# realphongha/UDP-Pose

Measured on AMD Instinct MI355X. Metric: images/sec HRNet-W32 256x192 (infer+decode), higher is better.
Workload: dtype f16x2 (split fp16 hi+lo operands = 22 bits, 3 fp16 MFMAs per product, fp32 accumulate); 1 GPU; w32 256x192 f16x2 inference, batch=64 per GPU, flip-test on, DARK decode (forward on 2N images + flip fuse + udp_decode_gaussian); global_batch=64, parallelism=replicas x1 (no data-path collective), weights=seeded synthetic, BN stats calibrated (tests/golden/bn_calib_w32_gaussian.npz)

## Files before the change

include/udp_pose_hip.h:

```cpp
#ifndef UDP_POSE_HIP_H
#define UDP_POSE_HIP_H

#include <stddef.h>
#include <stdint.h>

#ifdef __cplusplus
extern "C" {
#endif

#define UDP_POSE_ABI_VERSION 19

enum udp_status {
  UDP_OK = 0,
  UDP_ERR_ARG = -1,
  UDP_ERR_HIP = -2,
  UDP_ERR_UNSUPPORTED = -3,
  UDP_ERR_WORKSPACE = -4
};

enum udp_dtype { UDP_F32 = 0, UDP_BF16 = 1, UDP_F16X2 = 2 };

int udp_abi_version(void);
int udp_f16x2_overflow(void* stream, int reset);
const char* udp_last_error(void);
// ... 109 lines not shown
                          void* w_dgrad, void* stream);
typedef struct udp_pack_desc {
  const float* w;
  void* w_fwd;
  void* w_dgrad;
  int32_t cout, cin, ks, reserved;
} udp_pack_desc;
int udp_pack_conv_weights_batch(const udp_pack_desc* descs_dev, int n, int dtype, void* stream);
int udp_zero_stuff2(const void* dy, int n, int h, int w, int c, int dtype, void* out, void* stream);
size_t udp_conv2d_wgrad_workspace_bytes(int cout, int cin, int ks);
int udp_conv2d_wgrad(const void* x, const void* dy, int n, int hin, int win, int cin_k, int hout,
                     int wout, int cout_k, int ks, int stride, int cout, int cin, int dtype, float* dw,
                     int accumulate, void* workspace, size_t workspace_bytes, void* stream);
typedef struct udp_wgrad_item {
  const void* x;
  const void* dy;
  float* dw;
  void* workspace;
  size_t workspace_bytes;
  int32_t n, hin, win, cin_k, hout, wout, cout_k, ks, stride, cout, cin, accumulate;
} udp_wgrad_item;
int udp_debug_multi_order(const unsigned* tiles, const unsigned* ncby, const int* code, int n, unsigned cap,
                          unsigned* out_member, unsigned* out_tile, unsigned* out_cby, int* used_table);
int udp_conv2d_wgrad_group(const udp_wgrad_item* items, int n_items, int dtype, void* stream);
typedef struct udp_conv_item {
  const udp_conv_op* op;
  const void* in;
  const void* weights;
  const float* bias;
  const void* res;
  void* out;
  double* bn_ws;
  size_t bn_ws_doubles;
  int32_t bn_rows;
  int32_t reserved;
} udp_conv_item;
int udp_conv2d_fused_group(udp_conv_item* items, int n_items, int dtype, int n, void* stream);
size_t udp_bn_workspace_doubles(int c);
int udp_bn_train_fwd(const void* x, int64_t m, int c, const float* gamma, const float* beta, float eps,
                     float momentum, float* running_mean, float* running_var, float* save_mean,
                     float* save_invstd, const void* res, int relu, void* y, int dtype, double* ws,
                     void* stream);
int udp_bn_rows_max(void);
int udp_bn_train_fwd_from_sums(const void* x, int64_t m, int c, const float* gamma, const float* beta, float eps,
                               float momentum, float* running_mean, float* running_var, float* save_mean,
                               float* save_invstd, const void* res, int relu, void* y, int dtype, double* ws,
// ... 67 lines not shown
```

udp-pose_amd/_lib.py:

```python
import ctypes as C
import os

_HERE = os.path.dirname(os.path.abspath(__file__))
LIB_PATH = os.environ.get("UDP_POSE_LIB") or os.path.join(_HERE, "libudp_pose_hip.so")

UDP_OK = 0
UDP_F32, UDP_BF16, UDP_F16X2 = 0, 1, 2
DTYPES = {"f32": UDP_F32, "bf16": UDP_BF16, "f16x2": UDP_F16X2}
UDP_OP_STEM, UDP_OP_CONV, UDP_OP_FUSE, UDP_OP_STEM7, UDP_OP_MAXPOOL, UDP_OP_BILINEAR = 0, 1, 2, 3, 4, 5
UDP_OP_PSA_POOL, UDP_OP_PSA_MLP, UDP_OP_PSA_SCALE, UDP_OP_PSA_SP, UDP_OP_BLOCK = 6, 7, 8, 9, 10
UDP_OP_DECONV, UDP_OP_DWCONV, UDP_OP_PIXSHUF = 11, 12, 13
UDP_BUF_NONE, UDP_BUF_OUTPUT = -1, -2
ABI_VERSION = 19
MAX_LANES, MAX_WAIT = 4, 8


class BnItem(C.Structure):
    _fields_ = [(k, C.c_void_p) for k in ("x", "dy", "y_relu", "res", "y", "dx", "g_out", "gamma", "beta", "running_mean",
                                          "running_var", "save_mean", "save_invstd", "dgamma", "dbeta", "ws")] + [
        ("m", C.c_int64), ("c", C.c_int32), ("rows", C.c_int32), ("relu", C.c_int32), ("reserved", C.c_int32)]


class WgradItem(C.Structure):
    _fields_ = [("x", C.c_void_p), ("dy", C.c_void_p), ("dw", C.c_void_p), ("workspace", C.c_void_p),
# ... 77 lines not shown
                                     C.POINTER(C.c_float), C.POINTER(C.c_float), C.c_int, C.c_int, _P, _P]),
    "udp_aid_apply": (C.c_int, [_P, C.c_int, C.c_int, C.c_int, _P, C.c_int, _P, _P, C.c_int, C.c_int,
                                C.POINTER(C.c_float), C.POINTER(C.c_float), _P]),
    "udp_target_gaussian": (C.c_int, [_P, _P, C.c_int, C.c_int, C.c_int, C.c_int, C.c_int, C.c_int,
                                      C.c_float, _P, _P, _P]),
    "udp_target_offset": (C.c_int, [_P, _P, C.c_int, C.c_int, C.c_int, C.c_int, C.c_int, C.c_int,
                                    C.c_float, _P, _P, _P]),
    "udp_mse_loss": (C.c_int, [_P, _P, _P, C.c_int, C.c_int, C.c_int, C.c_int, _P, _P, _P]),
    "udp_oks_nms": (C.c_int, [_P, _P, _P, _P, C.POINTER(C.c_int32), C.c_int, C.c_int, _P, C.c_double, C.c_int,
                              C.c_double, C.c_int, C.c_double, C.c_int, _P, _P, _P]),
    "udp_pack_conv_weights": (C.c_int, [_P, C.c_int, C.c_int, C.c_int, C.c_int, _P, _P, _P]),
    "udp_pack_conv_weights_batch": (C.c_int, [_P, C.c_int, C.c_int, _P]),
    "udp_zero_stuff2": (C.c_int, [_P, C.c_int, C.c_int, C.c_int, C.c_int, C.c_int, _P, _P]),
    "udp_conv2d_wgrad_workspace_bytes": (C.c_size_t, [C.c_int, C.c_int, C.c_int]),
    "udp_conv2d_wgrad": (C.c_int, [_P, _P] + [C.c_int] * 12 + [_P, C.c_int, _P, C.c_size_t, _P]),
    "udp_bn_workspace_doubles": (C.c_size_t, [C.c_int]),
    "udp_bn_train_fwd": (C.c_int, [_P, C.c_int64, C.c_int, _P, _P, C.c_float, C.c_float, _P, _P, _P, _P, _P,
                                   C.c_int, _P, C.c_int, _P, _P]),
    "udp_bn_rows_max": (C.c_int, []),
    "udp_bn_train_fwd_from_sums": (C.c_int, [_P, C.c_int64, C.c_int, _P, _P, C.c_float, C.c_float, _P, _P, _P, _P, _P,
                                             C.c_int, _P, C.c_int, _P, C.c_int, _P]),
    "udp_bn_train_bwd": (C.c_int, [_P, _P, _P, C.c_int64, C.c_int, _P, _P, _P, _P, _P, _P, _P, C.c_int, _P, _P]),
    "udp_debug_multi_order": (C.c_int, [_P, _P, _P, C.c_int, C.c_uint, _P, _P, _P, _P]),
    "udp_conv2d_wgrad_group": (C.c_int, [_P, C.c_int, C.c_int, _P]),
    "udp_conv2d_fused_group": (C.c_int, [_P, C.c_int, C.c_int, C.c_int, _P]),
    "udp_bn_train_fwd_multi": (C.c_int, [_P, C.c_int, C.c_float, C.c_float, C.c_int, _P]),
    "udp_bn_train_bwd_multi": (C.c_int, [_P, C.c_int, C.c_int, _P]),
    "udp_ew_accumulate": (C.c_int, [_P, _P, C.c_int, C.c_int, C.c_int, C.c_int, C.c_int, C.c_int, C.c_int,
                                    C.c_int, _P]),
    "udp_relu_bwd": (C.c_int, [_P, _P, _P, C.c_int64, C.c_int, _P]),
    "udp_upsample_bwd": (C.c_int, [_P, C.c_int, C.c_int, C.c_int, C.c_int, C.c_int, _P, C.c_int, C.c_int, _P]),
    "udp_bias_grad": (C.c_int, [_P, C.c_int64, C.c_int, C.c_int, _P, C.c_int, _P]),
    "udp_nchw_to_nhwc": (C.c_int, [_P, C.c_int, C.c_int, C.c_int, C.c_int, C.c_int, _P, C.c_int, _P]),
    "udp_adam_step": (C.c_int, [_P, _P, _P, _P, C.c_int64, C.c_float, C.c_float, C.c_float, C.c_float, C.c_int,
                                C.c_float, _P]),
    "udp_adam_coefficients": (C.c_int, [C.c_float, C.c_float, C.c_float, C.c_int, _P]),
    "udp_adam_step_dev": (C.c_int, [_P, _P, _P, _P, C.c_int64, C.c_float, C.c_float, C.c_float, _P, C.c_float, _P]),
    "udp_psa_train_save_floats": (C.c_size_t, [C.c_int, C.c_int, C.c_int, C.c_int]),
    "udp_psa_train_fwd_pool": (C.c_int, [C.POINTER(PsaTrainArgs), C.c_int, _P]),
    "udp_psa_train_fwd_sp": (C.c_int, [C.POINTER(PsaTrainArgs), C.c_int, _P]),
    "udp_psa_train_bwd_sp": (C.c_int, [C.POINTER(PsaTrainArgs), C.c_int, _P]),
    "udp_psa_train_bwd_pool": (C.c_int, [C.POINTER(PsaTrainArgs), C.c_int, _P]),
    "udp_psa_train_bwd_params": (C.c_int, [C.POINTER(PsaTrainArgs), C.c_int, _P]),
}
EXPORTS = tuple(_SIGS)

# ... 42 lines not shown
```

udp-pose_amd/csrc/conv_dev.h:

```cpp
#pragma once
#include <cstdlib>
#include <type_traits>

#include "common.h"

namespace udp {


typedef float f32x4 __attribute__((ext_vector_type(4)));
typedef float f32x2 __attribute__((ext_vector_type(2)));
typedef __bf16 bf16x8 __attribute__((ext_vector_type(8)));
typedef __bf16 bf16x4 __attribute__((ext_vector_type(4)));
typedef _Float16 f16x8 __attribute__((ext_vector_type(8)));
typedef _Float16 f16x4 __attribute__((ext_vector_type(4)));

#ifndef UDP_H2_STORE_AUX
#define UDP_H2_STORE_AUX 0
#endif
#ifndef UDP_H2_RES_AUX
#define UDP_H2_RES_AUX 0
#endif
#ifndef UDP_H2_DMA_AUX
#define UDP_H2_DMA_AUX 0
#endif
// ... 237 lines not shown
      __builtin_amdgcn_raw_buffer_store_b128(__builtin_bit_cast(u32x4, v[nb]), r, voff + 16 * nb, 0, 0);
  } else if constexpr (std::is_same<T, H2>::value) {
#pragma unroll
    for (int h = 0; h < NB / 2; ++h) {
      f16x8 hi, lo;
      h2_split8(v[2 * h], v[2 * h + 1], hi, lo);
      __builtin_amdgcn_raw_buffer_store_b128(__builtin_bit_cast(u32x4, hi), r, voff + 16 * h, 0, UDP_H2_STORE_AUX);
      __builtin_amdgcn_raw_buffer_store_b128(__builtin_bit_cast(u32x4, lo), r, voff + lo_off + 16 * h, 0, UDP_H2_STORE_AUX);
    }
  } else {
#pragma unroll
    for (int h = 0; h < NB / 2; ++h) {
      bf16x8 o;
#pragma unroll
      for (int q = 0; q < 4; ++q) {
        o[q] = (__bf16)v[2 * h][q];
        o[4 + q] = (__bf16)v[2 * h + 1][q];
      }
      __builtin_amdgcn_raw_buffer_store_b128(__builtin_bit_cast(u32x4, o), r, voff + 16 * h, 0, 0);
    }
  }
}

static inline int largest_divisor_leq(int n, int lim) {
  for (int d = lim < n ? lim : n; d >= 1; --d)
    if (n % d == 0) return d;
  return 1;
}

}
```

udp-pose_amd/csrc/conv_ws.hip:

```cpp
#include "conv_dev.h"

namespace udp {

template <int NB>
struct ResH2 {
  u32x4 hi[NB / 2], lo[NB / 2];
};
template <int NB>
__device__ __forceinline__ void load_res_h2(ResH2<NB>& o, __amdgpu_buffer_rsrc_t r, unsigned voff, unsigned lo_off) {
#pragma unroll
  for (int h = 0; h < NB / 2; ++h) {
    o.hi[h] = __builtin_amdgcn_raw_buffer_load_b128(r, voff + 16 * h, 0, UDP_H2_RES_AUX);
    o.lo[h] = __builtin_amdgcn_raw_buffer_load_b128(r, voff + lo_off + 16 * h, 0, UDP_H2_RES_AUX);
  }
}
template <int NB>
__device__ __forceinline__ void add_res_h2(f32x4 (&v)[NB], const ResH2<NB>& o) {
#pragma unroll
  for (int h = 0; h < NB / 2; ++h) h2_add8(v[2 * h], v[2 * h + 1], __builtin_bit_cast(f16x8, o.hi[h]), __builtin_bit_cast(f16x8, o.lo[h]));
}

template <int KS, int STRIDE, int PB, int CP, bool NCHW, bool OUT2 = false>
__device__ __forceinline__ void conv_ws_body(const ConvParams& p, const int tile_id, const int cby) {
  using T = H2;
  constexpr int CK = 32, ESZ = 2, NB = 2, NW = 4;
  constexpr int PAD = KS / 2, TAPS = KS * KS;
  extern __shared__ __attribute__((aligned(16))) unsigned char smem[];

  UDP_STAMP(0);
  const int tid = threadIdx.x;
  const int lane = tid & 63;
  const int wave = __builtin_amdgcn_readfirstlane(tid >> 6);
  const int li = lane & 15;
  const int kg = lane >> 4;
  const int cp = wave % CP, pg = wave / CP;

  int t = tile_id;
  const int tx = t % p.tiles_x;
  t /= p.tiles_x;
  const int ty = t % p.tiles_y;
  const int n0 = (t / p.tiles_y) * p.G;
  const int y0 = ty * p.R;
  const int x0 = tx * p.TW;

  const int IH = p.IH, IW = p.IW;
  const int npix_in = p.G * IH * IW;
  const int in_groups = (npix_in + 15) >> 4;
  const int in_bytes = in_groups * 16 * ROWB;
  const int stage_bytes = 2 * in_bytes;
// ... 17 lines not shown
#else
  constexpr bool dbg_nost = false;
#endif
#if UDP_WS_DBG & 64
  const bool dbg_nores = nchunks == 1;
#else
  constexpr bool dbg_nores = false;
#endif
  const __amdgpu_buffer_rsrc_t r_out = __builtin_amdgcn_make_buffer_rsrc(
      p.out, 0, (!p.out || dbg_nost) ? 0 : NCHW ? out_pix * p.Cout * 4 : out_pix * outpb, 0x00020000);
  const __amdgpu_buffer_rsrc_t r_bias = __builtin_amdgcn_make_buffer_rsrc(
      const_cast<float*>(p.bias), 0, (unsigned)p.CoutPad * 4u, 0x00020000);
  const __amdgpu_buffer_rsrc_t r_res = __builtin_amdgcn_make_buffer_rsrc(
      const_cast<void*>(p.res), 0, (p.res && !dbg_nores) ? out_pix * respb : 0, 0x00020000);

  const int cwave = (cby * CP + cp) * 32;
  const int cbase = cwave + 8 * kg;
  const unsigned wvoff = (unsigned)lane * 16u;
  const unsigned wpair = (unsigned)(cby * CP + cp) * 4096u;
  constexpr int AD = UDP_WS_AD;
  f16x8 ah[AD][NB], al[AD][NB];
  const int nsteps = nchunks * TAPS;
  auto load_a = [&](int s, f16x8 (&h)[NB], f16x8 (&l)[NB]) __attribute__((always_inline)) {
    const int c = s / TAPS, tap = s - c * TAPS;
    const unsigned soff = (unsigned)(tap * nchunks + c) * (npairs * 4096u) + wpair;
#pragma unroll
    for (int nb = 0; nb < NB; ++nb) {
      h[nb] = __builtin_bit_cast(f16x8, __builtin_amdgcn_raw_buffer_load_b128(r_w, wvoff + 2048u * nb, soff, 0));
      l[nb] = __builtin_bit_cast(f16x8, __builtin_amdgcn_raw_buffer_load_b128(r_w, wvoff + 2048u * nb + 1024u, soff, 0));
    }
  };

#pragma unroll
  for (int k = 0; k < AD - 1; ++k) load_a(k < nsteps ? k : nsteps - 1, ah[k], al[k]);
  f32x4 bias[NB];
#pragma unroll
  for (int nb = 0; nb < NB; ++nb)
    bias[nb] = __builtin_bit_cast(f32x4, __builtin_amdgcn_raw_buffer_load_b128(r_bias, (unsigned)(cbase + 4 * nb) * 4u, 0, 0));

  const int srow = lane >> 2, spart = lane & 3;
  const int gy0 = y0 * STRIDE - PAD, gx0 = x0 * STRIDE - PAD;
  unsigned src_off[MAXG];
#pragma unroll
  for (int i = 0; i < MAXG; ++i) {
    unsigned off = kOobOff;
    if ((wave + NW * i) * 16 < npix_in) {
      const int row = (wave + NW * i) * 16 + srow;
      const int tmp = fdiv20(row, p.mIW);
      const int ix = row - (int)__umul24(tmp, IW);
      const int g = fdiv20(tmp, p.mIH);
      const int iy = tmp - (int)__umul24(g, IH);
      const int n = n0 + g, gy = gy0 + iy, gx = gx0 + ix;
      const bool ok = row < npix_in && n < p.N && (unsigned)gy < (unsigned)p.Hin && (unsigned)gx < (unsigned)p.Win;
      const unsigned pix = __umul24(__umul24(n, p.Hin) + gy, p.Win) + gx;
      off = ok ? pix * inpb + p.in_coff * ESZ + ((spart ^ swz<T>(row)) << 4) : kOobOff;
    }
    src_off[i] = off;
  }
  auto stage = [&](int c, unsigned char* sb) __attribute__((always_inline)) {
    const unsigned coff = (unsigned)c * (CK * ESZ);
    const bool cut = ragged && c == nchunks - 1;
    const int parts_left = (p.Cin - c * CK) / 8;
#pragma unroll
    for (int i = 0; i < MAXG; ++i) {
      const int gidx = wave + NW * i;
      if (gidx < in_groups) {
        unsigned off = src_off[i] + coff;
        if (cut && (spart ^ swz<T>(gidx * 16 + srow)) >= parts_left) off = kOobOff;
        blds16(r_in, off, sb + gidx * (16 * ROWB));
        blds16(r_in, off + in_lo, sb + in_bytes + gidx * (16 * ROWB));
      }
    }
  };

  UDP_STAMP(1);
  stage(0, smem);

  int prow[PB], opix[PB], ocrd[PB];
#pragma unroll
  for (int i = 0; i < PB; ++i) {
    const int m0 = (pg * PB + i) * 16 + li;
    const int m = m0 < M ? m0 : M - 1;
    const int g = fdiv20(m, p.mRT);
    const int rem = m - (int)__umul24(g, RT);
    const int r = fdiv20(rem, p.mTW);
    const int x = rem - (int)__umul24(r, p.TW);
    prow[i] = (int)__umul24(__umul24(g, IH) + r * STRIDE, IW) + x * STRIDE;
    const int n = n0 + g, y = y0 + r, xo = x0 + x;
    const bool ok = m0 < M && n < p.N && y < p.Hout && xo < p.Wout && (NCHW || cbase < p.Cout);
    const unsigned pix = __umul24(__umul24(n, p.Hout) + y, p.Wout) + xo;
    opix[i] = ok ? (int)pix : -1;
    ocrd[i] = ok ? (y | (xo << 10) | (n << 20)) : -1;
  }

  const float winv = __builtin_ldexpf(1.f, -p.wexp);
  f32x4 acc[PB][NB];
#pragma unroll
  for (int i = 0; i < PB; ++i)
#pragma unroll
    for (int nb = 0; nb < NB; ++nb) acc[i][nb] = f32x4{0.f, 0.f, 0.f, 0.f};

  constexpr int NR = NCHW ? 0 : PB * NB;
  ResH2<NB> rres[NCHW ? 1 : PB];
  __builtin_amdgcn_sched_barrier(0);
  asm volatile("" ::: "memory");
  if constexpr (!NCHW) {
#pragma unroll
    for (int i = 0; i < PB; ++i)
      load_res_h2(rres[i], r_res, opix[i] >= 0 ? (unsigned)opix[i] * respb + (p.res_coff + cbase) * ESZ : kOobOff, res_lo);
  }
  asm volatile("" ::: "memory");
  __builtin_amdgcn_sched_barrier(0);

  UDP_STAMP(2);
  int c = 0, tap = 0;
  const unsigned char* sb = smem;
  auto step = [&](auto BUFC, int s) __attribute__((always_inline)) {
    constexpr int BUF = decltype(BUFC)::value;
#if !(UDP_WS_DBG & 1)
    load_a(s + AD - 1 < nsteps ? s + AD - 1 : nsteps - 1, ah[(BUF + AD - 1) % AD], al[(BUF + AD - 1) % AD]);
#endif
    if (tap == 0) {
      if (c == 1) UDP_STAMP(9);
      if (c == 2) UDP_STAMP(11);
      if (c == 4) UDP_STAMP(13);
      bool refill = false;
      if constexpr (STRIDE == 2 || OUT2) refill = p.sbuf && c > 0;
      if (refill) {
        __syncthreads();
        stage(c, smem);
        asm volatile("s_waitcnt vmcnt(0)" ::: "memory");
        __syncthreads();
        sb = smem;
      } else {
        if (s == 0)
          asm volatile("s_waitcnt vmcnt(%0)" ::"n"(2 * NB + NR) : "memory");
        else
          asm volatile("s_waitcnt vmcnt(%0)" ::"n"(2 * NB) : "memory");
        if (s == 0) UDP_STAMP(3);
        __syncthreads();
        if (s == 0) UDP_STAMP(4);
        if (c == 1) UDP_STAMP(10);
        if (c == 2) UDP_STAMP(12);
        if (c == 4) UDP_STAMP(14);
#if !(UDP_WS_DBG & 4)
        if (c + 1 < nchunks && !((STRIDE == 2 || OUT2) && p.sbuf)) stage(c + 1, smem + ((c + 1) & 1) * stage_bytes);
#endif
        sb = smem + (c & 1) * stage_bytes;
      }
    }
    f16x8 a2[NB];
#pragma unroll
    for (int nb = 0; nb < NB; ++nb) a2[nb] = ah[BUF][nb] * (_Float16)0x1p-11f;
    const int tap_rows = KS == 1 ? 0 : (tap / KS) * IW + tap % KS;
    f16x8 xh[3], xl[3];
    auto load_b = [&](int i, f16x8& h, f16x8& l) __attribute__((always_inline)) {
      const int row = prow[i] + tap_rows;
      const unsigned char* q = sb + row * ROWB + ((kg ^ swz<T>(row)) << 4);
      h = *reinterpret_cast<const f16x8*>(q);
      l = *reinterpret_cast<const f16x8*>(q + in_bytes);
    };
    load_b(0, xh[0], xl[0]);
    if (PB > 1) load_b(1, xh[1], xl[1]);
#pragma unroll
    for (int i = 0; i < PB; ++i) {
#if !(UDP_WS_DBG & 2)
      if (i + 2 < PB) load_b(i + 2, xh[(i + 2) % 3], xl[(i + 2) % 3]);
#endif
      __builtin_amdgcn_sched_barrier(0);
#if UDP_WS_DBG & 16
      acc[i][0] = __builtin_amdgcn_mfma_f32_16x16x32_f16(ah[BUF][0] + al[BUF][1] + a2[0] + a2[1], xh[i % 3] + xl[i % 3], acc[i][0], 0, 0, 0);
#else
#pragma unroll
      for (int nb = 0; nb < NB; ++nb) acc[i][nb] = __builtin_amdgcn_mfma_f32_16x16x32_f16(ah[BUF][nb], xh[i % 3], acc[i][nb], 0, 0, 0);
#pragma unroll
      for (int nb = 0; nb < NB; ++nb) acc[i][nb] = __builtin_amdgcn_mfma_f32_16x16x32_f16(al[BUF][nb], xh[i % 3], acc[i][nb], 0, 0, 0);
#pragma unroll
      for (int nb = 0; nb < NB; ++nb) acc[i][nb] = __builtin_amdgcn_mfma_f32_16x16x32_f16(a2[nb], xl[i % 3], acc[i][nb], 0, 0, 0);
#endif
    }
    if (++tap == TAPS) {
      tap = 0;
      ++c;
    }
  };
  for (int s = 0; s < nsteps; s += AD) {
    step(std::integral_constant<int, 0>{}, s);
    if (s + 1 < nsteps) step(std::integral_constant<int, 1>{}, s + 1);
    if (s + 2 < nsteps) step(std::integral_constant<int, 2>{}, s + 2);
    if constexpr (AD > 3) if (s + 3 < nsteps) step(std::integral_constant<int, 3>{}, s + 3);
    if constexpr (AD > 4) if (s + 4 < nsteps) step(std::integral_constant<int, 4>{}, s + 4);
    if constexpr (AD > 5) if (s + 5 < nsteps) step(std::integral_constant<int, 5>{}, s + 5);
  }
  UDP_STAMP(5);
#pragma unroll
  for (int i = 0; i < PB; ++i) {
#pragma unroll
    for (int nb = 0; nb < NB; ++nb)
#pragma unroll
      for (int q = 0; q < 4; ++q) acc[i][nb][q] = __builtin_fmaf(acc[i][nb][q], winv, bias[nb][q]);
    if constexpr (!NCHW) add_res_h2(acc[i], rres[i]);
  }

#pragma unroll
  for (int i = 0; i < PB; ++i) {
    f32x4 v[NB];
// ... 76 lines not shown

__host__ __device__ __forceinline__ void ws_decode(unsigned b, unsigned ntiles, unsigned nc, int& tile, int& cby) {
  if (nc == 1) {
    tile = (int)b;
    cby = 0;
    return;
  }
  const unsigned full = (ntiles >> 3) * 8u * nc;
  unsigned base = 0, width = 8, r = b;
  if (b < full) {
    const unsigned g = b / (8u * nc);
    r = b - g * 8u * nc;
    base = g * 8u;
  } else {
    r = b - full;
    base = (ntiles >> 3) * 8u;
    width = ntiles & 7u;
  }
  const unsigned c = r / width;
  cby = (int)c;
  tile = (int)(base + r - c * width);
}

template <int KS, int STRIDE, int PB, int CP, bool NCHW>
__global__ __launch_bounds__(256, 2) void conv_ws_h2_kernel(const ConvParams p) {
  int tile, cby;
  ws_decode(blockIdx.x + gridDim.x * blockIdx.y, gridDim.x, gridDim.y, tile, cby);
  conv_ws_body<KS, STRIDE, PB, CP, NCHW, KS == 3 && STRIDE == 1 && !NCHW>(p, tile, cby);
}

#ifndef UDP_WS_MPB
#define UDP_WS_MPB 6
#define UDP_WS_MOCC 2
#endif
template <int KS>
__global__ __launch_bounds__(256, UDP_WS_MOCC) void conv_ws_multi(const ConvMulti m) {
  const unsigned b = blockIdx.x;
  int j, tile, cby;
  int code;
  const unsigned e = __builtin_amdgcn_readfirstlane(m.tab[(b >> 3) < (unsigned)kMultiTab ? (b >> 3) : 0u]);
  if (m.tab_n) {
    j = (int)(e & 3u);
    code = 1 << ((e >> 2) & 3u);
    cby = (int)((e >> 4) & 63u);
    tile = (int)((e >> 10) + (b & 7u));
  } else {
    int sg = 0;
#pragma unroll
    for (int k = 1; k < kMultiSegs; ++k) sg += b >= m.seg_start[k];
    j = __builtin_amdgcn_readfirstlane(m.seg_mem[sg]);
    const unsigned r = __builtin_amdgcn_readfirstlane(b - m.seg_start[sg] + m.seg_first[sg]);
    ws_decode(r, m.tiles[j], m.ncby[j], tile, cby);
    tile = __builtin_amdgcn_readfirstlane(tile);
    cby = __builtin_amdgcn_readfirstlane(cby);
    code = m.code[j];
  }
  switch (code) {
    case 1: conv_ws_body<KS, 1, UDP_WS_MPB, 1, false>(m.p[j], tile, (int)cby); break;
    case 2: conv_ws_body<KS, 1, UDP_WS_MPB, 2, false>(m.p[j], tile, (int)cby); break;
    default: conv_ws_body<KS, 1, UDP_WS_MPB, 4, false>(m.p[j], tile, (int)cby); break;
  }
}

template <int KS, int STRIDE, int PB, int CP, bool NCHW>
static int describe_ws_one(const ConvParams& p, size_t lds, Launch* out) {
  static bool attr_set = false;
  const void* kern = reinterpret_cast<const void*>(&conv_ws_h2_kernel<KS, STRIDE, PB, CP, NCHW>);
  if (!attr_set) {
    UDP_HIP_CHECK(hipFuncSetAttribute(kern, hipFuncAttributeMaxDynamicSharedMemorySize, 160 * 1024));
    attr_set = true;
  }
  out->fn = kern;
  out->grid = dim3(p.ntiles, p.CoutPad / (CP * 32));
  out->block = dim3(256);
  out->lds = (unsigned)lds;
  out->p = p;
  return UDP_OK;
}
template <int KS, int STRIDE, bool NCHW>
static int describe_ws_pb(const ConvParams& p, int pb, int cp, size_t lds, Launch* out) {
#define UDP_WS(B, C) \
  if (pb == B && cp == C) return describe_ws_one<KS, STRIDE, B, C, NCHW>(p, lds, out);
  UDP_WS(2, 1) UDP_WS(3, 1) UDP_WS(4, 1) UDP_WS(6, 1) UDP_WS(2, 2) UDP_WS(3, 2) UDP_WS(4, 2) UDP_WS(6, 2)
  UDP_WS(2, 4) UDP_WS(3, 4) UDP_WS(4, 4) UDP_WS(6, 4)
#undef UDP_WS
  return 1;
}
struct WsTile {
  int cp, pb, G, R, TW, wgs, sbuf;
  size_t lds;
};
static bool ws_tile(const ConvParams& p, int ks, int stride, int cp, int pb, WsTile* t, bool own_launch) {
  const int pg = 4 / cp;
  const int maxM = 16 * pb * pg;
  bool have = false;
  double best_util = 0.0;
  for (int split = 1; split <= 4 || !have; ++split) {
    if (split > 8) break;
    const int TW = ceil_div(p.Wout, split);
    if (TW > 64 || TW > maxM || (have && TW < 8)) continue;
    int maxR = maxM / TW;
    if (maxR > p.Hout) maxR = p.Hout;
    int R = largest_divisor_leq(p.Hout, maxR);
    if (R * 2 <= maxR) R = maxR;
    int G = 1;
    if (R == p.Hout && TW == p.Wout) {
      G = maxM / (R * TW);
      if (G > p.N) G = p.N;
      if (G < 1) G = 1;
    }
    auto npix = [&](int g, int r) { return g * ((r - 1) * stride + ks) * ((TW - 1) * stride + ks); };
    while (npix(G, R) > MAXG * 64 && G > 1) --G;
    while (npix(G, R) > MAXG * 64 && R > 1) R = (R + 1) / 2;
    if (npix(G, R) > MAXG * 64) continue;
    int nstage = ceil_div(p.Cin, 32) > 1 ? 2 : 1;
    size_t lds = (size_t)((npix(G, R) + 15) / 16) * 16 * ROWB * 2 * nstage;
    static const int sbuf_mode = getenv("UDP_POSE_WS_SBUF") == nullptr ? 1 : atoi(getenv("UDP_POSE_WS_SBUF"));
    const bool sbuf_kernel = stride == 2 || (ks == 3 && own_launch && sbuf_mode != 2);
    const bool sbuf = sbuf_kernel && nstage == 2 && lds > 80 * 1024 && lds / 2 <= 80 * 1024 && sbuf_mode != 0;
    if (sbuf) {
      nstage = 1;
      lds /= 2;
    }
    if (lds > 160 * 1024) continue;
    const int need = ceil_div(ceil_div(G * R * TW, 16), pg);
    if (need > pb) continue;
    const int pbe = need <= 2 ? 2 : need <= 3 ? 3 : need <= 4 ? 4 : 6;
    const int tiles = ceil_div(p.N, G) * ceil_div(p.Hout, R) * ceil_div(p.Wout, TW);
    const double util = (double)p.N * p.Hout * p.Wout / ((double)tiles * 16 * pbe * pg) *
                        ((double)G * R * TW * stride * stride / (double)npix(G, R));
    if (!have || util > best_util + 0.05) {
      have = true;
      best_util = util;
      t->cp = cp;
      t->pb = pbe;
      t->G = G;
      t->R = R;
      t->TW = TW;
      t->lds = lds;
      t->sbuf = sbuf ? 1 : 0;
      t->wgs = tiles * (p.CoutPad / (cp * 32));
    }
  }
  return have;
}

static long g_ws_fill_wgs = 512;
void ws_set_fill_wgs(long wgs) { g_ws_fill_wgs = wgs; }

int describe_conv_ws(ConvParams p, int ks, int stride, Launch* out, bool grouped) {
  if ((stride != 1 && stride != 2) || (ks != 3 && ks != 1) || (p.out_nchw_f32 && stride != 1))
    return fail(UDP_ERR_UNSUPPORTED, "fragment-major weights (wfmt 1): conv ks=%d stride=%d nchw_out=%d has no weight-stationary kernel",
                ks, stride, p.out_nchw_f32);
  auto knob = [](const char* name, long dflt) {
    const char* v = getenv(name);
    return v ? atol(v) : dflt;
  };
  const int pairs = p.CoutPad / 32;
  const int force_cp = (int)knob("UDP_POSE_WS_CP", 0), force_pb = (int)knob("UDP_POSE_WS_PB", 0);
  const long min_wgs = grouped ? 0 : knob("UDP_POSE_WS_MINWGS", g_ws_fill_wgs);
  WsTile best{}, t{};
  bool have = false;
  for (int pb : {6, 4, 3, 2}) {
    for (int cp : {4, 2, 1}) {
      if (pairs % cp || (force_cp && cp != force_cp) || (force_pb && pb != force_pb)) continue;
      if (grouped && stride == 1 && UDP_WS_MPB != 6 && pb != UDP_WS_MPB) continue;
      if (!ws_tile(p, ks, stride, cp, pb, &t, !grouped && !p.out_nchw_f32)) continue;
      const bool fills = t.wgs >= min_wgs, best_fills = have && best.wgs >= min_wgs;
      if (!have || (!best_fills && (fills || t.wgs > best.wgs))) {
        best = t;
        have = true;
      }
    }
  }
  if (!have) return fail(UDP_ERR_UNSUPPORTED, "weight-stationary conv: no tile for %dx%d C%d->%d", p.Hout, p.Wout, p.Cin, p.Cout);
  p.G = best.G;
  p.R = best.R;
  p.TW = best.TW;
  p.sbuf = best.sbuf;
  p.IH = (p.R - 1) * stride + ks;
  p.IW = (p.TW - 1) * stride + ks;
  p.tiles_x = ceil_div(p.Wout, p.TW);
  p.tiles_y = ceil_div(p.Hout, p.R);
  auto magic = [](int d) { return (unsigned)(((1u << 20) + (unsigned)d - 1) / (unsigned)d); };
  p.mIW = magic(p.IW);
  p.mIH = magic(p.IH);
  p.mRT = magic(p.R * p.TW);
  p.mTW = magic(p.TW);
  p.ntiles = ceil_div(p.N, p.G) * p.tiles_y * p.tiles_x;
  if (getenv("UDP_POSE_DEBUG_TILES"))
    fprintf(stderr, "ws conv k%d s%d %dx%d C%d->%d: G=%d R=%d TW=%d CP=%d PB=%d lds=%zu%s wgs=%d\n", ks, stride, p.Hout, p.Wout, p.Cin,
            p.Cout, p.G, p.R, p.TW, best.cp, best.pb, best.lds, best.sbuf ? " (one stage buffer)" : "", best.wgs);
  int rc = 1;
  if (ks == 3 && stride == 1 && !p.out_nchw_f32) rc = describe_ws_pb<3, 1, false>(p, best.pb, best.cp, best.lds, out);
  if (ks == 3 && stride == 1 && p.out_nchw_f32) rc = describe_ws_pb<3, 1, true>(p, best.pb, best.cp, best.lds, out);
  if (ks == 3 && stride == 2) rc = describe_ws_pb<3, 2, false>(p, best.pb, best.cp, best.lds, out);
  if (ks == 1 && stride == 1 && !p.out_nchw_f32) rc = describe_ws_pb<1, 1, false>(p, best.pb, best.cp, best.lds, out);
  if (ks == 1 && stride == 1 && p.out_nchw_f32) rc = describe_ws_pb<1, 1, true>(p, best.pb, best.cp, best.lds, out);
  if (ks == 1 && stride == 2) rc = describe_ws_pb<1, 2, false>(p, best.pb, best.cp, best.lds, out);
  if (rc == 1) return fail(UDP_ERR_UNSUPPORTED, "weight-stationary conv: no kernel for PB=%d CP=%d", best.pb, best.cp);
  if (rc == UDP_OK && p.nout2 && !(ks == 3 && stride == 1))
    return fail(UDP_ERR_UNSUPPORTED, "second outputs: 3x3 stride-1 convs only");
  if (rc == UDP_OK && grouped && best.pb == UDP_WS_MPB && stride == 1 && !p.nout2) {
    out->groupable = 300 + ks * 10 + 6;
    out->ws_cp = best.cp;
  }
  return rc;
}

static void ws_order(ConvMulti* m, int n) {
  struct Seg {
    unsigned start, first, cnt;
    int mem;
  };
  unsigned cnt_of[4];
  unsigned total = 0;
  for (int j = 0; j < n; ++j) {
    cnt_of[j] = (j + 1 < n ? m->start[j + 1] : m->start[4]) - m->start[j];
    total += cnt_of[j];
// ... 88 lines not shown
  ws_order(&m, n);
  if (used_table) *used_table = m.tab_n != 0;
  for (unsigned b = 0; b < total; ++b) {
    int j, tile, cby;
    if (m.tab_n) {
      const unsigned e = m.tab[b >> 3];
      j = (int)(e & 3u);
      if ((1 << ((e >> 2) & 3u)) != m.code[j]) return -1;
      cby = (int)((e >> 4) & 63u);
      tile = (int)((e >> 10) + (b & 7u));
    } else {
      int sg = 0;
      for (int k = 1; k < kMultiSegs; ++k) sg += b >= m.seg_start[k];
      j = m.seg_mem[sg];
      ws_decode(b - m.seg_start[sg] + m.seg_first[sg], m.tiles[j], m.ncby[j], tile, cby);
    }
    out_member[b] = (unsigned)j;
    out_tile[b] = (unsigned)tile;
    out_cby[b] = (unsigned)cby;
  }
  return (int)total;
}

int describe_ws_multi(const Launch* members, int n, ConvMulti* m, Launch* out) {
  static bool ws_attr_set = false;
  const void* wk[2] = {reinterpret_cast<const void*>(&conv_ws_multi<3>), reinterpret_cast<const void*>(&conv_ws_multi<1>)};
  if (!ws_attr_set) {
    for (const void* k : wk) UDP_HIP_CHECK(hipFuncSetAttribute(k, hipFuncAttributeMaxDynamicSharedMemorySize, 160 * 1024));
    ws_attr_set = true;
  }
  memset(m, 0, sizeof(*m));
  unsigned total = 0, lds = 0;
  for (int j = 0; j < n; ++j) {
    if (members[j].groupable != members[0].groupable) return fail(UDP_ERR_ARG, "describe_multi: mixed weight-stationary members");
    m->p[j] = members[j].p;
    m->start[j] = total;
    m->tiles[j] = members[j].grid.x;
    m->ncby[j] = members[j].grid.y;
    m->code[j] = members[j].ws_cp;
    total += members[j].grid.x * members[j].grid.y;
    if (members[j].lds > lds) lds = members[j].lds;
  }
  for (int j = n; j < 5; ++j) m->start[j] = j < 4 ? 0xFFFFFFFFu : total;
  for (int j = n; j < 4; ++j) m->tiles[j] = m->ncby[j] = 1;
  ws_order(m, n);
  out->fn = wk[members[0].groupable / 10 % 10 == 3 ? 0 : 1];
// ... 255 lines not shown
```

Before: 8186 images/s.

## Stream 3x3 stride-2 conv input tiles by parity phase in weight-stationary kernel

Adds a phase-streamed path for 3x3 stride-2 convolutions. The input tile is split into four parity phases, each of size (R+1)x(TW+1). Taps are reordered so each phase is staged and consumed in turn, with double buffering across phases and channel chunks. The aim is to shrink the LDS footprint and avoid staging the padded strided halo, which allows larger output tiles or two workgroups per CU. In exchange it adds more barriers and staging rounds per chunk, plus new tile-selection logic and debug entry points.

```diff
diff --git a/include/udp_pose_hip.h b/include/udp_pose_hip.h
--- a/include/udp_pose_hip.h
+++ b/include/udp_pose_hip.h
@@ -155,6 +155,8 @@
 } udp_wgrad_item;
 int udp_debug_multi_order(const unsigned* tiles, const unsigned* ncby, const int* code, int n, unsigned cap,
                           unsigned* out_member, unsigned* out_tile, unsigned* out_cby, int* used_table);
+int udp_debug_s2_geom(int n_img, int hin, int win, int G, int R, int TW, int tile, int cap_rows, int* stage, int* reads);
+int udp_debug_s2_tile(int n_img, int hin, int win, int cin, int cout, int* out);
 int udp_conv2d_wgrad_group(const udp_wgrad_item* items, int n_items, int dtype, void* stream);
 typedef struct udp_conv_item {
   const udp_conv_op* op;
diff --git a/udp-pose_amd/_lib.py b/udp-pose_amd/_lib.py
--- a/udp-pose_amd/_lib.py
+++ b/udp-pose_amd/_lib.py
@@ -123,6 +123,8 @@
                                              C.c_int, _P, C.c_int, _P, C.c_int, _P]),
     "udp_bn_train_bwd": (C.c_int, [_P, _P, _P, C.c_int64, C.c_int, _P, _P, _P, _P, _P, _P, _P, C.c_int, _P, _P]),
     "udp_debug_multi_order": (C.c_int, [_P, _P, _P, C.c_int, C.c_uint, _P, _P, _P, _P]),
+    "udp_debug_s2_geom": (C.c_int, [C.c_int] * 8 + [_P, _P]),
+    "udp_debug_s2_tile": (C.c_int, [C.c_int] * 5 + [_P]),
     "udp_conv2d_wgrad_group": (C.c_int, [_P, C.c_int, C.c_int, _P]),
     "udp_conv2d_fused_group": (C.c_int, [_P, C.c_int, C.c_int, C.c_int, _P]),
     "udp_bn_train_fwd_multi": (C.c_int, [_P, C.c_int, C.c_float, C.c_float, C.c_int, _P]),
diff --git a/udp-pose_amd/csrc/conv_dev.h b/udp-pose_amd/csrc/conv_dev.h
--- a/udp-pose_amd/csrc/conv_dev.h
+++ b/udp-pose_amd/csrc/conv_dev.h
@@ -283,6 +283,32 @@
   }
 }
 
+constexpr int kS2Steps = 9;
+__host__ __device__ __forceinline__ int s2_tap_of_step(int k) { return (int)((0x453718620ull >> (4 * k)) & 15u); }
+__host__ __device__ __forceinline__ bool s2_step_opens_phase(int k) { return (0x151u >> k) & 1u; }
+__host__ __device__ __forceinline__ int s2_phase_of_step(int k) { return (k >= 4) + (k >= 6) + (k >= 8); }
+__host__ __device__ __forceinline__ int s2_phase_of_tap(int tap) { return ((tap / 3 == 1) << 1) | (tap % 3 == 1); }
+constexpr int kS2PhaseMajor = 1;
+__host__ __device__ __forceinline__ void s2_step_ck(int s, int n, int pm, int& c, int& k) {
+  if (!pm) {
+    c = s / kS2Steps;
+    k = s - c * kS2Steps;
+    return;
+  }
+  const int ph = (s >= 4 * n) + (s >= 6 * n) + (s >= 8 * n);
+  const int k0 = (0x8640 >> (4 * ph)) & 15, lg = (0x0112 >> (4 * ph)) & 3;
+  const int r = s - k0 * n;
+  c = r >> lg;
+  k = k0 + (r & ((1 << lg) - 1));
+}
+__host__ __device__ __forceinline__ bool s2_stage_line(int p, int j, int o0, int T, int lim, int& g) {
+  g = 2 * (o0 + j) - 1 + p;
+  return j <= T - p && g >= 0 && g < lim;
+}
+__host__ __device__ __forceinline__ int s2_read_row(int r, int x, int tap, int IW) {
+  return (r + (tap / 3 == 2)) * IW + x + (tap % 3 == 2);
+}
+
 static inline int largest_divisor_leq(int n, int lim) {
   for (int d = lim < n ? lim : n; d >= 1; --d)
     if (n % d == 0) return d;
diff --git a/udp-pose_amd/csrc/conv_ws.hip b/udp-pose_amd/csrc/conv_ws.hip
--- a/udp-pose_amd/csrc/conv_ws.hip
+++ b/udp-pose_amd/csrc/conv_ws.hip
@@ -20,11 +20,12 @@
   for (int h = 0; h < NB / 2; ++h) h2_add8(v[2 * h], v[2 * h + 1], __builtin_bit_cast(f16x8, o.hi[h]), __builtin_bit_cast(f16x8, o.lo[h]));
 }
 
-template <int KS, int STRIDE, int PB, int CP, bool NCHW, bool OUT2 = false>
+template <int KS, int STRIDE, int PB, int CP, bool NCHW, bool OUT2 = false, bool PH = false>
 __device__ __forceinline__ void conv_ws_body(const ConvParams& p, const int tile_id, const int cby) {
   using T = H2;
   constexpr int CK = 32, ESZ = 2, NB = 2, NW = 4;
   constexpr int PAD = KS / 2, TAPS = KS * KS;
+  static_assert(!PH || (KS == 3 && STRIDE == 2 && !OUT2), "phase streaming: 3x3 stride-2 convs");
   extern __shared__ __attribute__((aligned(16))) unsigned char smem[];
 
   UDP_STAMP(0);
@@ -88,7 +89,11 @@
   f16x8 ah[AD][NB], al[AD][NB];
   const int nsteps = nchunks * TAPS;
   auto load_a = [&](int s, f16x8 (&h)[NB], f16x8 (&l)[NB]) __attribute__((always_inline)) {
-    const int c = s / TAPS, tap = s - c * TAPS;
+    int c = s / TAPS, tap = s - c * TAPS;
+    if constexpr (PH) {
+      s2_step_ck(s, nchunks, kS2PhaseMajor, c, tap);
+      tap = s2_tap_of_step(tap);
+    }
     const unsigned soff = (unsigned)(tap * nchunks + c) * (npairs * 4096u) + wpair;
 #pragma unroll
     for (int nb = 0; nb < NB; ++nb) {
@@ -107,6 +112,7 @@
   const int srow = lane >> 2, spart = lane & 3;
   const int gy0 = y0 * STRIDE - PAD, gx0 = x0 * STRIDE - PAD;
   unsigned src_off[MAXG];
+  unsigned okr[2] = {0u, 0u}, okc[2] = {0u, 0u};
 #pragma unroll
   for (int i = 0; i < MAXG; ++i) {
     unsigned off = kOobOff;
@@ -116,6 +122,19 @@
       const int ix = row - (int)__umul24(tmp, IW);
       const int g = fdiv20(tmp, p.mIH);
       const int iy = tmp - (int)__umul24(g, IH);
+      if constexpr (PH) {
+        const int n = n0 + g;
+        const bool img = row < npix_in && n < p.N;
+        int y3 = 0, x3 = 0;
+#pragma unroll
+        for (int q = 0; q < 2; ++q) {
+          okr[q] |= (unsigned)(s2_stage_line(q, iy, y0, p.R, p.Hin, y3) && img) << i;
+          okc[q] |= (unsigned)(s2_stage_line(q, ix, x0, p.TW, p.Win, x3) && img) << i;
+        }
+        const unsigned pix = __umul24(__umul24(n, p.Hin) + y3, p.Win) + x3;
+        src_off[i] = pix * inpb + p.in_coff * ESZ + ((spart ^ swz<T>(row)) << 4);
+        continue;
+      }
       const int n = n0 + g, gy = gy0 + iy, gx = gx0 + ix;
       const bool ok = row < npix_in && n < p.N && (unsigned)gy < (unsigned)p.Hin && (unsigned)gx < (unsigned)p.Win;
       const unsigned pix = __umul24(__umul24(n, p.Hin) + gy, p.Win) + gx;
@@ -139,8 +158,27 @@
     }
   };
 
+  auto stage_ph = [&](int c, int ph, unsigned char* sb) __attribute__((always_inline)) {
+    const int pr = ph >> 1, pc = ph & 1;
+    const unsigned coff = (unsigned)c * (CK * ESZ) - (unsigned)((1 - pr) * p.Win + (1 - pc)) * inpb;
+    const unsigned okm = okr[pr] & okc[pc];
+    const bool cut = ragged && c == nchunks - 1;
+    const int parts_left = (p.Cin - c * CK) / 8;
+#pragma unroll
+    for (int i = 0; i < MAXG; ++i) {
+      const int gidx = wave + NW * i;
+      if (gidx < in_groups) {
+        unsigned off = ((okm >> i) & 1u) ? src_off[i] + coff : kOobOff;
+        if (cut && (spart ^ swz<T>(gidx * 16 + srow)) >= parts_left) off = kOobOff;
+        blds16(r_in, off, sb + gidx * (16 * ROWB));
+        blds16(r_in, off + in_lo, sb + in_bytes + gidx * (16 * ROWB));
+      }
+    }
+  };
+
   UDP_STAMP(1);
-  stage(0, smem);
+  if constexpr (PH) stage_ph(0, 0, smem);
+  else stage(0, smem);
 
   int prow[PB], opix[PB], ocrd[PB];
 #pragma unroll
@@ -151,7 +189,8 @@
     const int rem = m - (int)__umul24(g, RT);
     const int r = fdiv20(rem, p.mTW);
     const int x = rem - (int)__umul24(r, p.TW);
-    prow[i] = (int)__umul24(__umul24(g, IH) + r * STRIDE, IW) + x * STRIDE;
+    prow[i] = PH ? (int)__umul24(__umul24(g, IH), IW) + s2_read_row(r, x, 0, IW)
+                 : (int)__umul24(__umul24(g, IH) + r * STRIDE, IW) + x * STRIDE;
     const int n = n0 + g, y = y0 + r, xo = x0 + x;
     const bool ok = m0 < M && n < p.N && y < p.Hout && xo < p.Wout && (NCHW || cbase < p.Cout);
     const unsigned pix = __umul24(__umul24(n, p.Hout) + y, p.Wout) + xo;
@@ -186,7 +225,23 @@
 #if !(UDP_WS_DBG & 1)
     load_a(s + AD - 1 < nsteps ? s + AD - 1 : nsteps - 1, ah[(BUF + AD - 1) % AD], al[(BUF + AD - 1) % AD]);
 #endif
-    if (tap == 0) {
+    if constexpr (PH) {
+      constexpr int pm = kS2PhaseMajor;
+      s2_step_ck(s, nchunks, pm, c, tap);
+      if (s2_step_opens_phase(tap)) {
+        const int ph = s2_phase_of_step(tap);
+        if (s == 0)
+          asm volatile("s_waitcnt vmcnt(%0)" ::"n"(2 * NB + NR) : "memory");
+        else
+          asm volatile("s_waitcnt vmcnt(%0)" ::"n"(2 * NB) : "memory");
+        __syncthreads();
+        const int u = pm ? ph * nchunks + c : c * 4 + ph;
+        const bool wrap = pm ? c + 1 == nchunks : ph == 3;
+        const int cn = pm ? (wrap ? 0 : c + 1) : (wrap ? c + 1 : c), pn = pm ? (wrap ? ph + 1 : ph) : (ph + 1) & 3;
+        if (u + 1 < nchunks * 4) stage_ph(cn, pn, smem + ((u + 1) & 1) * stage_bytes);
+        sb = smem + (u & 1) * stage_bytes;
+      }
+    } else if (tap == 0) {
       if (c == 1) UDP_STAMP(9);
       if (c == 2) UDP_STAMP(11);
       if (c == 4) UDP_STAMP(13);
@@ -218,7 +273,7 @@
     f16x8 a2[NB];
 #pragma unroll
     for (int nb = 0; nb < NB; ++nb) a2[nb] = ah[BUF][nb] * (_Float16)0x1p-11f;
-    const int tap_rows = KS == 1 ? 0 : (tap / KS) * IW + tap % KS;
+    const int tap_rows = KS == 1 ? 0 : PH ? s2_read_row(0, 0, s2_tap_of_step(tap), IW) : (tap / KS) * IW + tap % KS;
     f16x8 xh[3], xl[3];
     auto load_b = [&](int i, f16x8& h, f16x8& l) __attribute__((always_inline)) {
       const int row = prow[i] + tap_rows;
@@ -245,9 +300,11 @@
       for (int nb = 0; nb < NB; ++nb) acc[i][nb] = __builtin_amdgcn_mfma_f32_16x16x32_f16(a2[nb], xl[i % 3], acc[i][nb], 0, 0, 0);
 #endif
     }
-    if (++tap == TAPS) {
-      tap = 0;
-      ++c;
+    if constexpr (!PH) {
+      if (++tap == TAPS) {
+        tap = 0;
+        ++c;
+      }
     }
   };
   for (int s = 0; s < nsteps; s += AD) {
@@ -370,11 +427,11 @@
   tile = (int)(base + r - c * width);
 }
 
-template <int KS, int STRIDE, int PB, int CP, bool NCHW>
+template <int KS, int STRIDE, int PB, int CP, bool NCHW, bool PH = false>
 __global__ __launch_bounds__(256, 2) void conv_ws_h2_kernel(const ConvParams p) {
   int tile, cby;
   ws_decode(blockIdx.x + gridDim.x * blockIdx.y, gridDim.x, gridDim.y, tile, cby);
-  conv_ws_body<KS, STRIDE, PB, CP, NCHW, KS == 3 && STRIDE == 1 && !NCHW>(p, tile, cby);
+  conv_ws_body<KS, STRIDE, PB, CP, NCHW, KS == 3 && STRIDE == 1 && !NCHW, PH>(p, tile, cby);
 }
 
 #ifndef UDP_WS_MPB
@@ -410,10 +467,10 @@
   }
 }
 
-template <int KS, int STRIDE, int PB, int CP, bool NCHW>
+template <int KS, int STRIDE, int PB, int CP, bool NCHW, bool PH = false>
 static int describe_ws_one(const ConvParams& p, size_t lds, Launch* out) {
   static bool attr_set = false;
-  const void* kern = reinterpret_cast<const void*>(&conv_ws_h2_kernel<KS, STRIDE, PB, CP, NCHW>);
+  const void* kern = reinterpret_cast<const void*>(&conv_ws_h2_kernel<KS, STRIDE, PB, CP, NCHW, PH>);
   if (!attr_set) {
     UDP_HIP_CHECK(hipFuncSetAttribute(kern, hipFuncAttributeMaxDynamicSharedMemorySize, 160 * 1024));
     attr_set = true;
@@ -425,10 +482,10 @@
   out->p = p;
   return UDP_OK;
 }
-template <int KS, int STRIDE, bool NCHW>
+template <int KS, int STRIDE, bool NCHW, bool PH = false>
 static int describe_ws_pb(const ConvParams& p, int pb, int cp, size_t lds, Launch* out) {
 #define UDP_WS(B, C) \
-  if (pb == B && cp == C) return describe_ws_one<KS, STRIDE, B, C, NCHW>(p, lds, out);
+  if (pb == B && cp == C) return describe_ws_one<KS, STRIDE, B, C, NCHW, PH>(p, lds, out);
   UDP_WS(2, 1) UDP_WS(3, 1) UDP_WS(4, 1) UDP_WS(6, 1) UDP_WS(2, 2) UDP_WS(3, 2) UDP_WS(4, 2) UDP_WS(6, 2)
   UDP_WS(2, 4) UDP_WS(3, 4) UDP_WS(4, 4) UDP_WS(6, 4)
 #undef UDP_WS
@@ -438,7 +495,8 @@
   int cp, pb, G, R, TW, wgs, sbuf;
   size_t lds;
 };
-static bool ws_tile(const ConvParams& p, int ks, int stride, int cp, int pb, WsTile* t, bool own_launch) {
+constexpr size_t kWsLdsTwoWgs = 80 * 1024;
+static bool ws_tile(const ConvParams& p, int ks, int stride, int cp, int pb, WsTile* t, bool own_launch, bool phased = false) {
   const int pg = 4 / cp;
   const int maxM = 16 * pb * pg;
   bool have = false;
@@ -457,14 +515,16 @@
       if (G > p.N) G = p.N;
       if (G < 1) G = 1;
     }
-    auto npix = [&](int g, int r) { return g * ((r - 1) * stride + ks) * ((TW - 1) * stride + ks); };
-    while (npix(G, R) > MAXG * 64 && G > 1) --G;
-    while (npix(G, R) > MAXG * 64 && R > 1) R = (R + 1) / 2;
-    if (npix(G, R) > MAXG * 64) continue;
-    int nstage = ceil_div(p.Cin, 32) > 1 ? 2 : 1;
-    size_t lds = (size_t)((npix(G, R) + 15) / 16) * 16 * ROWB * 2 * nstage;
+    auto npix = [&](int g, int r) { return phased ? g * (r + 1) * (TW + 1) : g * ((r - 1) * stride + ks) * ((TW - 1) * stride + ks); };
+    auto stage_lds = [&](int g, int r) { return (size_t)((npix(g, r) + 15) / 16) * 16 * ROWB * 2; };
+    auto fits = [&](int g, int r) { return npix(g, r) <= MAXG * 64 && (!phased || 2 * stage_lds(g, r) <= kWsLdsTwoWgs); };
+    while (!fits(G, R) && G > 1) --G;
+    while (!fits(G, R) && R > 1) R = (R + 1) / 2;
+    if (!fits(G, R)) continue;
+    int nstage = phased || ceil_div(p.Cin, 32) > 1 ? 2 : 1;
+    size_t lds = stage_lds(G, R) * nstage;
     static const int sbuf_mode = getenv("UDP_POSE_WS_SBUF") == nullptr ? 1 : atoi(getenv("UDP_POSE_WS_SBUF"));
-    const bool sbuf_kernel = stride == 2 || (ks == 3 && own_launch && sbuf_mode != 2);
+    const bool sbuf_kernel = !phased && (stride == 2 || (ks == 3 && own_launch && sbuf_mode != 2));
     const bool sbuf = sbuf_kernel && nstage == 2 && lds > 80 * 1024 && lds / 2 <= 80 * 1024 && sbuf_mode != 0;
     if (sbuf) {
       nstage = 1;
@@ -476,7 +536,7 @@
     const int pbe = need <= 2 ? 2 : need <= 3 ? 3 : need <= 4 ? 4 : 6;
     const int tiles = ceil_div(p.N, G) * ceil_div(p.Hout, R) * ceil_div(p.Wout, TW);
     const double util = (double)p.N * p.Hout * p.Wout / ((double)tiles * 16 * pbe * pg) *
-                        ((double)G * R * TW * stride * stride / (double)npix(G, R));
+                        ((double)G * R * TW * (phased ? 1 : stride * stride) / (double)npix(G, R));
     if (!have || util > best_util + 0.05) {
       have = true;
       best_util = util;
@@ -496,14 +556,14 @@
 static long g_ws_fill_wgs = 512;
 void ws_set_fill_wgs(long wgs) { g_ws_fill_wgs = wgs; }
 
-int describe_conv_ws(ConvParams p, int ks, int stride, Launch* out, bool grouped) {
-  if ((stride != 1 && stride != 2) || (ks != 3 && ks != 1) || (p.out_nchw_f32 && stride != 1))
-    return fail(UDP_ERR_UNSUPPORTED, "fragment-major weights (wfmt 1): conv ks=%d stride=%d nchw_out=%d has no weight-stationary kernel",
-                ks, stride, p.out_nchw_f32);
+constexpr int kS2PhasedMinPixels = 32 * 24;
+static bool ws_choose(const ConvParams& p, int ks, int stride, bool grouped, WsTile* chosen, bool* phased_out) {
   auto knob = [](const char* name, long dflt) {
     const char* v = getenv(name);
     return v ? atol(v) : dflt;
   };
+  const long ph_knob = knob("UDP_POSE_WS_S2_PHASED", -1);
+  const bool phased = ks == 3 && stride == 2 && (ph_knob < 0 ? p.Hout * p.Wout >= kS2PhasedMinPixels : ph_knob != 0);
   const int pairs = p.CoutPad / 32;
   const int force_cp = (int)knob("UDP_POSE_WS_CP", 0), force_pb = (int)knob("UDP_POSE_WS_PB", 0);
   const long min_wgs = grouped ? 0 : knob("UDP_POSE_WS_MINWGS", g_ws_fill_wgs);
@@ -513,7 +573,7 @@
     for (int cp : {4, 2, 1}) {
       if (pairs % cp || (force_cp && cp != force_cp) || (force_pb && pb != force_pb)) continue;
       if (grouped && stride == 1 && UDP_WS_MPB != 6 && pb != UDP_WS_MPB) continue;
-      if (!ws_tile(p, ks, stride, cp, pb, &t, !grouped && !p.out_nchw_f32)) continue;
+      if (!ws_tile(p, ks, stride, cp, pb, &t, !grouped && !p.out_nchw_f32, phased)) continue;
       const bool fills = t.wgs >= min_wgs, best_fills = have && best.wgs >= min_wgs;
       if (!have || (!best_fills && (fills || t.wgs > best.wgs))) {
         best = t;
@@ -521,13 +581,25 @@
       }
     }
   }
-  if (!have) return fail(UDP_ERR_UNSUPPORTED, "weight-stationary conv: no tile for %dx%d C%d->%d", p.Hout, p.Wout, p.Cin, p.Cout);
+  *chosen = best;
+  *phased_out = phased;
+  return have;
+}
+
+int describe_conv_ws(ConvParams p, int ks, int stride, Launch* out, bool grouped) {
+  if ((stride != 1 && stride != 2) || (ks != 3 && ks != 1) || (p.out_nchw_f32 && stride != 1))
+    return fail(UDP_ERR_UNSUPPORTED, "fragment-major weights (wfmt 1): conv ks=%d stride=%d nchw_out=%d has no weight-stationary kernel",
+                ks, stride, p.out_nchw_f32);
+  WsTile best{};
+  bool phased = false;
+  if (!ws_choose(p, ks, stride, grouped, &best, &phased))
+    return fail(UDP_ERR_UNSUPPORTED, "weight-stationary conv: no tile for %dx%d C%d->%d", p.Hout, p.Wout, p.Cin, p.Cout);
   p.G = best.G;
   p.R = best.R;
   p.TW = best.TW;
   p.sbuf = best.sbuf;
-  p.IH = (p.R - 1) * stride + ks;
-  p.IW = (p.TW - 1) * stride + ks;
+  p.IH = phased ? p.R + 1 : (p.R - 1) * stride + ks;
+  p.IW = phased ? p.TW + 1 : (p.TW - 1) * stride + ks;
   p.tiles_x = ceil_div(p.Wout, p.TW);
   p.tiles_y = ceil_div(p.Hout, p.R);
   auto magic = [](int d) { return (unsigned)(((1u << 20) + (unsigned)d - 1) / (unsigned)d); };
@@ -538,11 +610,12 @@
   p.ntiles = ceil_div(p.N, p.G) * p.tiles_y * p.tiles_x;
   if (getenv("UDP_POSE_DEBUG_TILES"))
     fprintf(stderr, "ws conv k%d s%d %dx%d C%d->%d: G=%d R=%d TW=%d CP=%d PB=%d lds=%zu%s wgs=%d\n", ks, stride, p.Hout, p.Wout, p.Cin,
-            p.Cout, p.G, p.R, p.TW, best.cp, best.pb, best.lds, best.sbuf ? " (one stage buffer)" : "", best.wgs);
+            p.Cout, p.G, p.R, p.TW, best.cp, best.pb, best.lds, best.sbuf ? " (one stage buffer)" : phased ? " (phase-streamed)" : "", best.wgs);
   int rc = 1;
   if (ks == 3 && stride == 1 && !p.out_nchw_f32) rc = describe_ws_pb<3, 1, false>(p, best.pb, best.cp, best.lds, out);
   if (ks == 3 && stride == 1 && p.out_nchw_f32) rc = describe_ws_pb<3, 1, true>(p, best.pb, best.cp, best.lds, out);
-  if (ks == 3 && stride == 2) rc = describe_ws_pb<3, 2, false>(p, best.pb, best.cp, best.lds, out);
+  if (ks == 3 && stride == 2 && !phased) rc = describe_ws_pb<3, 2, false>(p, best.pb, best.cp, best.lds, out);
+  if (ks == 3 && stride == 2 && phased) rc = describe_ws_pb<3, 2, false, true>(p, best.pb, best.cp, best.lds, out);
   if (ks == 1 && stride == 1 && !p.out_nchw_f32) rc = describe_ws_pb<1, 1, false>(p, best.pb, best.cp, best.lds, out);
   if (ks == 1 && stride == 1 && p.out_nchw_f32) rc = describe_ws_pb<1, 1, true>(p, best.pb, best.cp, best.lds, out);
   if (ks == 1 && stride == 2) rc = describe_ws_pb<1, 2, false>(p, best.pb, best.cp, best.lds, out);
@@ -677,6 +750,69 @@
   return (int)total;
 }
 
+extern "C" int udp_debug_s2_geom(int n_img, int hin, int win, int G, int R, int TW, int tile, int cap_rows, int* stage, int* reads) {
+  if (n_img < 1 || hin < 1 || win < 1 || G < 1 || R < 1 || TW < 1 || tile < 0 || !stage || !reads) return -1;
+  const int hout = (hin - 1) / 2 + 1, wout = (win - 1) / 2 + 1;
+  const int tiles_x = ceil_div(wout, TW), tiles_y = ceil_div(hout, R);
+  if (tile >= ceil_div(n_img, G) * tiles_y * tiles_x) return -1;
+  const int IH = R + 1, IW = TW + 1, rows = G * IH * IW;
+  if (rows > cap_rows) return -1;
+  const int x0 = (tile % tiles_x) * TW, y0 = (tile / tiles_x % tiles_y) * R, n0 = (tile / tiles_x / tiles_y) * G;
+  for (int ph = 0; ph < 4; ++ph)
+    for (int row = 0; row < rows; ++row) {
+      const int i = row % IW, j = row / IW % IH, g = row / IW / IH;
+      int gy, gx;
+      const bool rok = s2_stage_line(ph >> 1, j, y0, R, hin, gy), cok = s2_stage_line(ph & 1, i, x0, TW, win, gx);
+      int* o = stage + ((size_t)ph * rows + row) * 4;
+      o[0] = n0 + g;
+      o[1] = gy;
+      o[2] = gx;
+      o[3] = rok && cok && n0 + g < n_img;
+    }
+  for (int m = 0; m < G * R * TW; ++m)
+    for (int k = 0; k < kS2Steps; ++k) {
+      const int tap = s2_tap_of_step(k);
+      const int x = m % TW, r = m / TW % R, g = m / TW / R;
+      reads[(m * 9 + tap) * 2] = s2_phase_of_tap(tap);
+      reads[(m * 9 + tap) * 2 + 1] = g * IH * IW + s2_read_row(r, x, tap, IW);
+      if (s2_phase_of_step(k) != s2_phase_of_tap(tap)) return -1;
+    }
+  for (int pm = 0; pm < 2; ++pm)
+    for (int n = 1; n <= 12; ++n) {
+      unsigned seen[12] = {0};
+      int pc = 0, pk = -1;
+      for (int s = 0; s < kS2Steps * n; ++s) {
+        int c, k;
+        s2_step_ck(s, n, pm, c, k);
+        if (c < 0 || c >= n || k < 0 || k >= kS2Steps || ((seen[c] >> k) & 1u)) return -1;
+        seen[c] |= 1u << k;
+        const bool same_stage = c == pc && pk >= 0 && s2_phase_of_step(k) == s2_phase_of_step(pk);
+        if (same_stage ? k != pk + 1 : !s2_step_opens_phase(k)) return -1;
+        pc = c;
+        pk = k;
+      }
+    }
+  return rows;
+}
+extern "C" int udp_debug_s2_tile(int n_img, int hin, int win, int cin, int cout, int* out) {
+  if (n_img < 1 || hin < 1 || win < 1 || cin < 1 || cout < 1 || !out) return -1;
+  ConvParams p{};
+  p.N = n_img;
+  p.Hin = hin;
+  p.Win = win;
+  p.Cin = cin;
+  p.Hout = (hin - 1) / 2 + 1;
+  p.Wout = (win - 1) / 2 + 1;
+  p.Cout = cout;
+  p.CoutPad = ceil_div(cout, 32) * 32;
+  WsTile t{};
+  bool phased = false;
+  if (!ws_choose(p, 3, 2, false, &t, &phased)) return -1;
+  const int v[8] = {t.G, t.R, t.TW, t.pb, t.cp, (int)t.lds, phased ? 1 : 0, t.wgs};
+  for (int k = 0; k < 8; ++k) out[k] = v[k];
+  return 0;
+}
+
 int describe_ws_multi(const Launch* members, int n, ConvMulti* m, Launch* out) {
   static bool ws_attr_set = false;
   const void* wk[2] = {reinterpret_cast<const void*>(&conv_ws_multi<3>), reinterpret_cast<const void*>(&conv_ws_multi<1>)};
```

Result: no change. 8259 images/s, median of 6 (+0.9%).
